# pyannote/pyannote-video

Hardware: AMD Instinct MI355X
Metric: frames/sec end-to-end detect->embed->cluster, 1080p@25fps (higher is better)
Workload: dtype f32 (detector scores, embedder) / f64 (tracker, clustering) / u8 frames; an f16 screening pass with a proven error bound decides which windows the detector's exact f32 chain is evaluated for -- results identical to dense f32 scoring (`dense_scoring`)

## Files before the change

### pyannote-video_amd/csrc/ert.hip

```cpp
#include "pvf_internal.h"

struct ErtJob { const uint8_t* img; int h, w; int rect[4]; };

__global__ void __launch_bounds__(256) ert_k(const ErtJob* __restrict__ jobs, int n_cascades, int n_trees, int n_parts, int n_pix, int depth,
                                             const float* __restrict__ initial, const int32_t* __restrict__ anchor,
                                             const float* __restrict__ deltas, const int32_t* __restrict__ idx1,
                                             const int32_t* __restrict__ idx2, const float* __restrict__ thresh,
                                             const float* __restrict__ leaves, int32_t* __restrict__ pts)
{
    extern __shared__ __attribute__((aligned(16))) float smem[];
    const int P2 = 2 * n_parts;
    float* cur = smem;
    float* pix = cur + ((P2 + 3) & ~3);
    int* leaf = reinterpret_cast<int*>(pix + ((n_pix + 3) & ~3));
    __shared__ float M[4];
    const ErtJob job = jobs[blockIdx.x];
    const int tid = threadIdx.x;
    const int n_split = (1 << depth) - 1, n_leaf = 1 << depth;
    const double sx = (double)job.rect[2] - (double)job.rect[0], sy = (double)job.rect[3] - (double)job.rect[1];
    const double ox = job.rect[0], oy = job.rect[1];
    for (int k = tid; k < P2; k += blockDim.x) cur[k] = initial[k];
    for (int it = 0; it < n_cascades; ++it) {
        __syncthreads();
        if (tid == 0) {
            double mfx = 0, mfy = 0, mtx = 0, mty = 0;
            for (int i = 0; i < n_parts; ++i) { mfx += initial[2 * i]; mfy += initial[2 * i + 1]; mtx += cur[2 * i]; mty += cur[2 * i + 1]; }
            mfx /= n_parts; mfy /= n_parts; mtx /= n_parts; mty /= n_parts;
            double a = 0, b = 0, s = 0;
            for (int i = 0; i < n_parts; ++i) {
                const double fx = initial[2 * i] - mfx, fy = initial[2 * i + 1] - mfy;
                const double tx = cur[2 * i] - mtx, ty = cur[2 * i + 1] - mty;
                a += fx * tx + fy * ty;
                b += fx * ty - fy * tx;
                s += fx * fx + fy * fy;
            }
            const double ca = a / s, cb = b / s;
            M[0] = (float)ca; M[1] = (float)(-cb); M[2] = (float)cb; M[3] = (float)ca;
        }
        __syncthreads();
        const int32_t* an = anchor + (size_t)it * n_pix;
        const float* dl = deltas + (size_t)it * n_pix * 2;
        for (int i = tid; i < n_pix; i += blockDim.x) {
            const float dx = dl[2 * i], dy = dl[2 * i + 1];
            const int ai = an[i];
            const float u = (M[0] * dx + M[1] * dy) + cur[2 * ai];
            const float v = (M[2] * dx + M[3] * dy) + cur[2 * ai + 1];
            const double X = (double)u * sx + ox, Y = (double)v * sy + oy;
            const long px = (long)floor(X + 0.5), py = (long)floor(Y + 0.5);
            float val = 0.0f;
            if (px >= 0 && py >= 0 && px < job.w && py < job.h) {
                const uint8_t* p = job.img + ((size_t)py * job.w + px) * 3;
                val = (float)(((unsigned)p[0] + p[1] + p[2]) / 3);
            }
            pix[i] = val;
        }
        __syncthreads();
        for (int t = tid; t < n_trees; t += blockDim.x) {
            const size_t sb = ((size_t)it * n_trees + t) * n_split;
            int i = 0;
            while (i < n_split) {
                if (pix[idx1[sb + i]] - pix[idx2[sb + i]] > thresh[sb + i]) i = 2 * i + 1;
                else i = 2 * i + 2;
            }
            leaf[t] = i - n_split;
        }
        __syncthreads();
        for (int k = tid; k < P2; k += blockDim.x) {
            float acc = cur[k];
            const float* lb = leaves + (size_t)it * n_trees * n_leaf * P2 + k;
            int t = 0;
            for (; t + 20 <= n_trees; t += 20) {
                float v[20];
#pragma unroll
                for (int j = 0; j < 20; ++j) v[j] = lb[((size_t)(t + j) * n_leaf + leaf[t + j]) * P2];
#pragma unroll
                for (int j = 0; j < 20; ++j) acc = acc + v[j];
            }
            for (; t < n_trees; ++t) acc = acc + lb[((size_t)t * n_leaf + leaf[t]) * P2];
            cur[k] = acc;
        }
    }
    __syncthreads();
    for (int i = tid; i < n_parts; i += blockDim.x) {
        const double X = (double)cur[2 * i] * sx + ox, Y = (double)cur[2 * i + 1] * sy + oy;
        pts[((size_t)blockIdx.x * n_parts + i) * 2] = (int32_t)floor(X + 0.5);
        pts[((size_t)blockIdx.x * n_parts + i) * 2 + 1] = (int32_t)floor(Y + 0.5);
    }
}

void ert_run(Ctx* c, const std::vector<Frame>& frames, const pvf_rect_i32* boxes, int n, int32_t* pts)
{
    const ShapeModel& s = c->shape;
    PVF_REQUIRE(s.loaded, "shape predictor not loaded");
    if (n == 0) return;
    std::vector<ErtJob> jobs(n);
    for (int i = 0; i < n; ++i) {
        jobs[i].img = frames[i].d; jobs[i].h = frames[i].h; jobs[i].w = frames[i].w;
        jobs[i].rect[0] = boxes[i].left; jobs[i].rect[1] = boxes[i].top; jobs[i].rect[2] = boxes[i].right; jobs[i].rect[3] = boxes[i].bottom;
    }
    ScratchLayout lay;
    const auto sJobs = lay.take<ErtJob>(n, 64); const auto sPts = lay.take<int32_t>((size_t)n * s.n_parts * 2, 64);
    lay.pad(64);
    c->s_misc.ensure(lay.bytes());
    ErtJob* d_jobs = sJobs.in(c->s_misc); int32_t* d_pts = sPts.in(c->s_misc);
    HIP_CHECK(hipMemcpyAsync(d_jobs, jobs.data(), sJobs.bytes(), hipMemcpyHostToDevice, c->stream));
    const size_t lds = (size_t)(((2 * s.n_parts + 3) & ~3) + ((s.n_pix + 3) & ~3)) * 4 + (size_t)s.n_trees * 4;
    {
        ProfScope ps(c, "ert");
        hipLaunchKernelGGL(ert_k, dim3(n), dim3(256), lds, c->stream, d_jobs, s.n_cascades, s.n_trees,
                           s.n_parts, s.n_pix, s.depth, s.d_initial, s.d_anchor, s.d_deltas, s.d_idx1, s.d_idx2, s.d_thresh, s.d_leaves,
                           d_pts);
    }
    HIP_CHECK(hipGetLastError());
    HIP_CHECK(hipMemcpyAsync(pts, d_pts, sPts.bytes(), hipMemcpyDeviceToHost, c->stream));
    HIP_CHECK(hipStreamSynchronize(c->stream));
}
```

### pyannote-video_amd/csrc/resnet.hip

```cpp
#include "pvf_internal.h"
#include <cmath>
#include <cstdlib>
#include <cstring>
#include <vector>

typedef float f32x4 __attribute__((ext_vector_type(4)));
typedef uint32_t u32x4 __attribute__((ext_vector_type(4)));
typedef float f32x16 __attribute__((ext_vector_type(16)));
typedef _Float16 f16x8 __attribute__((ext_vector_type(8)));
typedef _Float16 f16x4 __attribute__((ext_vector_type(4)));
typedef uint32_t u32x2 __attribute__((ext_vector_type(2)));

void face_chip_details(const EmbedModel& m, const int32_t* pts, ChipDetails* out)
{
    const double size = m.chip_size, padding = m.chip_padding;
    double fx[51], fy[51], tx[51], ty[51];
    int n = 0;
    for (int i = 17; i < 68; ++i) {
        if ((55 <= i && i <= 59) || (65 <= i && i <= 67)) continue;
        if (17 <= i && i <= 26) continue;
        fx[n] = ((padding + (double)m.mean_shape[2 * (i - 17)]) / (2 * padding + 1)) * size;
        fy[n] = ((padding + (double)m.mean_shape[2 * (i - 17) + 1]) / (2 * padding + 1)) * size;
        tx[n] = pts[2 * i]; ty[n] = pts[2 * i + 1];
        ++n;
    }
    double mfx = 0, mfy = 0, mtx = 0, mty = 0;
    for (int i = 0; i < n; ++i) { mfx += fx[i]; mfy += fy[i]; mtx += tx[i]; mty += ty[i]; }
    mfx /= n; mfy /= n; mtx /= n; mty /= n;
    double a = 0, b = 0, s = 0;
    for (int i = 0; i < n; ++i) {
        const double ax = fx[i] - mfx, ay = fy[i] - mfy, bx = tx[i] - mtx, by = ty[i] - mty;
        a += ax * bx + ay * by;
        b += ax * by - ay * bx;
        s += ax * ax + ay * ay;
    }
    const double ca = a / s, cb = b / s;
    const double scale = std::sqrt(ca * ca + cb * cb);
    const double hx = size / 2.0, hy = size / 2.0;
    const double cx = (ca * (hx - mfx) - cb * (hy - mfy)) + mtx;
    const double cy = (cb * (hx - mfx) + ca * (hy - mfy)) + mty;
    const double wv = size * scale;
    out->l = cx - wv / 2; out->t = cy - wv / 2; out->r = cx + wv / 2; out->b = cy + wv / 2;
    out->cs = ca / scale; out->sn = cb / scale;
    out->rows = m.chip_size; out->cols = m.chip_size;
}

struct ConvArgs {
    const float* in; int B, H, W, Cin;
    const float* w; int K;
    const float* frag;
    const float* bias; const float* gamma; const float* beta;
    float* out; int OH, OW, Cout;
    int AH, AW;
    int ksz, stride, pad;
    int skip_mode;
    const float* skip; int XH, XW, XC, SH, SW;
    const uint32_t* wsplit; float out_scale; int* flags;
};


__device__ __forceinline__ int small_div(int x, int d, float rd)
{
    int q = (int)((float)x * rd);
    const int r = x - q * d;
    q += (r >= d) ? 1 : 0;
    q -= (r < 0) ? 1 : 0;
    return q;
}

template <int WM, int WN>
__device__ __forceinline__ void conv_epilogue(const ConvArgs& a, float* smem, const f32x16& acc0, const f32x16& acc1, long M, long m0, int n0,
                                              int rel0, int b_first, int hw, float r_hw, float r_ow, int wave, int lane)
{
    constexpr int PITCH = 36;
    const int wm = wave / WN, wn = wave % WN;
    const int li = lane & 31, kh = lane >> 5;
    const int col = n0 + wn * 32 + li;
    const float bias = a.bias[col], g = a.gamma[col], bt = a.beta[col];
    if (a.AH == a.OH && a.AW == a.OW && a.skip_mode != 2) {
        float* T = smem + wave * 64 * PITCH;
#pragma unroll
        for (int t = 0; t < 2; ++t)
#pragma unroll
            for (int reg = 0; reg < 16; ++reg)
                T[(t * 32 + (reg & 3) + 8 * (reg >> 2) + 4 * kh) * PITCH + li] = (t == 0 ? acc0[reg] : acc1[reg]);
        __builtin_amdgcn_wave_barrier();
        const int c4 = lane & 7, cb = n0 + wn * 32 + 4 * c4;
        const float4 bias4 = *reinterpret_cast<const float4*>(a.bias + cb), g4 = *reinterpret_cast<const float4*>(a.gamma + cb),
                     bt4 = *reinterpret_cast<const float4*>(a.beta + cb);
#pragma unroll
        for (int it = 0; it < 8; ++it) {
            const int row = it * 8 + (lane >> 3);
            const long m = m0 + wm * 64 + row;
            if (m >= M) continue;
            const float4 x = *reinterpret_cast<const float4*>(&T[row * PITCH + 4 * c4]);
            float4 v = make_float4((x.x + bias4.x) * g4.x + bt4.x, (x.y + bias4.y) * g4.y + bt4.y, (x.z + bias4.z) * g4.z + bt4.z,
                                   (x.w + bias4.w) * g4.w + bt4.w);
            if (a.skip_mode == 1) {
                const float4 sk = *reinterpret_cast<const float4*>(a.skip + (size_t)m * a.Cout + cb);
                v.x += sk.x; v.y += sk.y; v.z += sk.z; v.w += sk.w;
            }
            { v.x = v.x < 0.0f ? 0.0f : v.x; v.y = v.y < 0.0f ? 0.0f : v.y; v.z = v.z < 0.0f ? 0.0f : v.z; v.w = v.w < 0.0f ? 0.0f : v.w; }
            *reinterpret_cast<float4*>(a.out + (size_t)m * a.Cout + cb) = v;
        }
        return;
    }
#pragma unroll
    for (int t = 0; t < 2; ++t)
#pragma unroll
        for (int reg = 0; reg < 16; ++reg) {
            const int row = (reg & 3) + 8 * (reg >> 2) + 4 * kh;
            const long m = m0 + wm * 64 + t * 32 + row;
            if (m >= M) continue;
            const int rel = rel0 + wm * 64 + t * 32 + row;
            const int bb = small_div(rel, hw, r_hw);
            const int rem = rel - bb * hw;
            const int oy = small_div(rem, a.OW, r_ow);
            const int ox = rem - oy * a.OW;
            const int b = b_first + bb;
            float v = 0.0f;
            if (oy < a.AH && ox < a.AW) v = ((t == 0 ? acc0[reg] : acc1[reg]) + bias) * g + bt;
            if (a.skip_mode == 1) v += a.skip[(size_t)m * a.Cout + col];
            else if (a.skip_mode == 2) {
                if (col < a.XC && oy < a.SH && ox < a.SW) {
                    const float* q = a.skip + (((size_t)b * a.XH + 2 * oy) * a.XW + 2 * ox) * a.XC + col;
                    v += (((q[0] + q[a.XC]) + q[(size_t)a.XW * a.XC]) + q[(size_t)a.XW * a.XC + a.XC]) * 0.25f;
                }
            }
            if (v < 0.0f) v = 0.0f;
            a.out[(size_t)m * a.Cout + col] = v;
        }
}

struct ConvExact {
    static constexpr bool FLAGS = false;
    static constexpr int LANE_K = 16;
    static __device__ __forceinline__ const u32x4* weights(const ConvArgs& a) { return reinterpret_cast<const u32x4*>(a.w); }
    static __device__ __forceinline__ bool park_a(uint32_t* row, int j4, const u32x4& v)
    {
        *reinterpret_cast<uint2*>(row + 2 * j4) = make_uint2(v.x, v.z);
        *reinterpret_cast<uint2*>(row + 2 * j4 + 16) = make_uint2(v.y, v.w);
        return true;
    }
    static __device__ __forceinline__ void park_b(uint32_t* row, int j4, const u32x4& v) { park_a(row, j4, v); }
    static __device__ __forceinline__ void chunk(const uint32_t* pa0, const uint32_t* pa1, const uint32_t* pb, f32x16& acc0, f32x16& acc1)
    {
        f32x4 fa0[4], fa1[4], fb[4];
#pragma unroll
        for (int q = 0; q < 4; ++q) {
            fa0[q] = *reinterpret_cast<const f32x4*>(pa0 + 4 * q);
            fa1[q] = *reinterpret_cast<const f32x4*>(pa1 + 4 * q);
            fb[q] = *reinterpret_cast<const f32x4*>(pb + 4 * q);
        }
#pragma unroll
        for (int s = 0; s < 16; ++s) {
            acc0 = __builtin_amdgcn_mfma_f32_32x32x2f32(fa0[s >> 2][s & 3], fb[s >> 2][s & 3], acc0, 0, 0, 0);
            acc1 = __builtin_amdgcn_mfma_f32_32x32x2f32(fa1[s >> 2][s & 3], fb[s >> 2][s & 3], acc1, 0, 0, 0);
        }
    }
    static __device__ __forceinline__ void scale(const ConvArgs&, f32x16&, f32x16&) {}
};

#define EMB_A_SCALE_EXP 8
#define EMB_F16_LIMIT 65504.0f
struct ConvSplit {
    static constexpr bool FLAGS = true;
    static constexpr int LANE_K = 4;
    static __device__ __forceinline__ const u32x4* weights(const ConvArgs& a) { return reinterpret_cast<const u32x4*>(a.wsplit); }
    static __device__ __forceinline__ bool park_a(uint32_t* row, int j4, const u32x4& v)
    {
        const f32x4 xv = __builtin_bit_cast(f32x4, v) * (float)(1 << EMB_A_SCALE_EXP);
        const bool ok = __builtin_reduce_and(__builtin_elementwise_abs(xv) < EMB_F16_LIMIT);
        const f16x4 hi = __builtin_convertvector(xv, f16x4), lo = __builtin_convertvector(xv - __builtin_convertvector(hi, f32x4), f16x4);
        *reinterpret_cast<u32x2*>(row + 2 * j4) = __builtin_bit_cast(u32x2, hi);
        *reinterpret_cast<u32x2*>(row + 2 * j4 + 16) = __builtin_bit_cast(u32x2, lo);
        return ok;
    }
    static __device__ __forceinline__ void park_b(uint32_t* row, int j4, const u32x4& v) { *reinterpret_cast<u32x4*>(row + 4 * j4) = v; }
    static __device__ __forceinline__ void chunk(const uint32_t* pa0, const uint32_t* pa1, const uint32_t* pb, f32x16& acc0, f32x16& acc1)
    {
#pragma unroll
        for (int s = 0; s < 2; ++s) {
            const f16x8 ah0 = *reinterpret_cast<const f16x8*>(pa0 + 8 * s), al0 = *reinterpret_cast<const f16x8*>(pa0 + 16 + 8 * s);
            const f16x8 ah1 = *reinterpret_cast<const f16x8*>(pa1 + 8 * s), al1 = *reinterpret_cast<const f16x8*>(pa1 + 16 + 8 * s);
            const f16x8 bh = *reinterpret_cast<const f16x8*>(pb + 8 * s), bl = *reinterpret_cast<const f16x8*>(pb + 16 + 8 * s);
            acc0 = __builtin_amdgcn_mfma_f32_32x32x16_f16(ah0, bh, acc0, 0, 0, 0);
            acc1 = __builtin_amdgcn_mfma_f32_32x32x16_f16(ah1, bh, acc1, 0, 0, 0);
            acc0 = __builtin_amdgcn_mfma_f32_32x32x16_f16(ah0, bl, acc0, 0, 0, 0);
            acc1 = __builtin_amdgcn_mfma_f32_32x32x16_f16(ah1, bl, acc1, 0, 0, 0);
            acc0 = __builtin_amdgcn_mfma_f32_32x32x16_f16(al0, bh, acc0, 0, 0, 0);
            acc1 = __builtin_amdgcn_mfma_f32_32x32x16_f16(al1, bh, acc1, 0, 0, 0);
        }
    }
    static __device__ __forceinline__ void scale(const ConvArgs& a, f32x16& acc0, f32x16& acc1) { acc0 *= a.out_scale; acc1 *= a.out_scale; }
};

template <int WM, int WN, class Ops>
__global__ void __launch_bounds__(256) conv_tile_k(ConvArgs a)
{
    constexpr int BM = 64 * WM, BN = 32 * WN, KC = 32, PITCH = 36;
    static_assert(WM * WN == 4, "four waves per block");
    constexpr int SM_ROWS = (BM + BN > 256) ? BM + BN : 256;
    __shared__ __attribute__((aligned(16))) float smem[SM_ROWS * PITCH];
    uint32_t* As = reinterpret_cast<uint32_t*>(smem);
    uint32_t* Bs = As + BM * PITCH;
    const int tid = threadIdx.x, lane = tid & 63, wave = tid >> 6;
    const int wm = wave / WN, wn = wave % WN;
    const long M = (long)a.B * a.OH * a.OW;
    const long m0 = (long)blockIdx.x * BM;
    const int n0 = blockIdx.y * BN;
    f32x16 acc0, acc1;
#pragma unroll
    for (int i = 0; i < 16; ++i) { acc0[i] = 0.0f; acc1[i] = 0.0f; }

    constexpr int A_F4 = BM * 8 / 256, B_F4 = BN * 8 / 256;
    constexpr int RSRC_FLAGS = 0x00020000, OOB = (int)0x80000000;
    const int hw = a.OH * a.OW;
    const int b_first = (int)(m0 / hw);
    const int rel0 = (int)(m0 - (long)b_first * hw);
    const float r_hw = 1.0f / (float)hw, r_ow = 1.0f / (float)a.OW;
    const size_t face = (size_t)a.H * a.W * a.Cin;
    const size_t in_bytes = (size_t)(a.B - b_first) * face * sizeof(float);
    const __amdgpu_buffer_rsrc_t rs_in = __builtin_amdgcn_make_buffer_rsrc((void*)(a.in + (size_t)b_first * face), 0,
                                                                           in_bytes > 0x7ffffff0u ? 0x7ffffff0 : (int)in_bytes, RSRC_FLAGS);
    int pa_off[A_F4], pa_y[A_F4], pa_x[A_F4];
#pragma unroll
    for (int q = 0; q < A_F4; ++q) {
        const int i = (tid + q * 256) >> 3;
        const long m = m0 + i;
        pa_off[q] = 0; pa_y[q] = -(1 << 20); pa_x[q] = 0;
        if (m < M) {
            const int rel = rel0 + i;
            const int bb = small_div(rel, hw, r_hw);
            const int rem = rel - bb * hw;
            const int oy = small_div(rem, a.OW, r_ow);
            const int ox = rem - oy * a.OW;
            if (oy < a.AH && ox < a.AW) {
                pa_y[q] = oy * a.stride - a.pad; pa_x[q] = ox * a.stride - a.pad;
                pa_off[q] = ((bb * a.H + pa_y[q]) * a.W + pa_x[q]) * a.Cin;
            }
        }
    }
    const int Kpad = (a.K + KC - 1) / KC * KC;
    const int j4 = tid & 7;
    const u32x4* wrow[B_F4];
#pragma unroll
    for (int q = 0; q < B_F4; ++q) wrow[q] = Ops::weights(a) + (size_t)(n0 + ((tid + q * 256) >> 3)) * (Kpad / 4) + j4;
    u32x4 va[A_F4], vb[B_F4];
    int f_r = 0, f_s = 0, f_c = 0, f_k = 0;
    int voff[A_F4], woff = 0;
    auto offsets = [&]() {
        const int kq = f_k + 4 * j4;
        const int r = f_r, sft = f_s;
        const int delta = (r * a.W + sft) * a.Cin + f_c + 4 * j4;
        const int k_ok = (kq < a.K) ? -1 : 0;
#pragma unroll
        for (int q = 0; q < A_F4; ++q) {
            const int iy = pa_y[q] + r, ix = pa_x[q] + sft;
            const int ok = k_ok & -(int)((unsigned)iy < (unsigned)a.H) & -(int)((unsigned)ix < (unsigned)a.W);
            voff[q] = (((pa_off[q] + delta) * 4) & ok) | (OOB & ~ok);
        }
        woff = f_k >> 2;
        if (f_k + KC < Kpad) {
            f_k += KC;
            f_c += KC;
            if (f_c >= a.Cin) { f_c = 0; if (++f_s == a.ksz) { f_s = 0; ++f_r; } }
        }
    };
    auto issue = [&]() {
#pragma unroll
        for (int q = 0; q < A_F4; ++q) va[q] = __builtin_amdgcn_raw_buffer_load_b128(rs_in, voff[q], 0, 0);
#pragma unroll
        for (int q = 0; q < B_F4; ++q) vb[q] = wrow[q][woff];
    };
    auto park = [&]() {
        int bad = 0;
#pragma unroll
        for (int q = 0; q < A_F4; ++q) bad |= Ops::park_a(&As[((tid + q * 256) >> 3) * PITCH], j4, va[q]) ? 0 : (1 << q);
#pragma unroll
        for (int q = 0; q < B_F4; ++q) Ops::park_b(&Bs[((tid + q * 256) >> 3) * PITCH], j4, vb[q]);
        if constexpr (Ops::FLAGS)
            if (bad)
                for (int q = 0; q < A_F4; ++q)
                    if ((bad >> q) & 1) a.flags[b_first + small_div(rel0 + ((tid + q * 256) >> 3), hw, r_hw)] = 1;
    };
    const int li = lane & 31, kh = lane >> 5;
    const uint32_t* pa0 = &As[(wm * 64 + li) * PITCH + Ops::LANE_K * kh];
    const uint32_t* pa1 = pa0 + 32 * PITCH;
    const uint32_t* pb = &Bs[(wn * 32 + li) * PITCH + Ops::LANE_K * kh];
    offsets();
    issue();
    offsets();
    for (int k0 = 0; k0 < Kpad; k0 += KC) {
        park();
        __syncthreads();
        issue();
        __builtin_amdgcn_sched_barrier(0);
        offsets();
        Ops::chunk(pa0, pa1, pb, acc0, acc1);
        __syncthreads();
    }
    Ops::scale(a, acc0, acc1);
    conv_epilogue<WM, WN>(a, smem, acc0, acc1, M, m0, n0, rel0, b_first, hw, r_hw, r_ow, wave, lane);
}


__global__ void __launch_bounds__(256) conv_wsplit_k(const float* __restrict__ w, int total, int w_exp, _Float16* __restrict__ out)
{
    const int i = blockIdx.x * 256 + threadIdx.x;
    if (i >= total) return;
    const float v = ldexpf(w[i], w_exp);
    const _Float16 hi = (_Float16)v;
    const _Float16 lo = (_Float16)(v - (float)hi);
    const int row32 = i >> 5, kk = i & 31;
    out[(size_t)row32 * 64 + kk] = hi;
    out[(size_t)row32 * 64 + 32 + kk] = lo;
}

__global__ void __launch_bounds__(64) embed_probe_k(const uint4* __restrict__ a, const uint4* __restrict__ b, int steps, float* __restrict__ d)
{
    const int lane = threadIdx.x;
    f32x16 acc;
#pragma unroll
    for (int i = 0; i < 16; ++i) acc[i] = 0.0f;
    for (int s = 0; s < steps; ++s)
        acc = __builtin_amdgcn_mfma_f32_32x32x16_f16(__builtin_bit_cast(f16x8, a[s * 64 + lane]), __builtin_bit_cast(f16x8, b[s * 64 + lane]), acc, 0, 0, 0);
    for (int i = 0; i < 16; ++i) d[lane * 16 + i] = acc[i];
}

#define STEM_ROWS 4
#define STEM_IN_DW 1464
#define STEM_NP 77
__global__ void __launch_bounds__(64) stem_frag_k(const float* __restrict__ w, float* __restrict__ frag)
{
    const int p = blockIdx.x, l = threadIdx.x;
    const int r = p / 11, t = 2 * (p - r * 11) + (l >> 5);
    frag[p * 64 + l] = (t < 21) ? w[(size_t)(l & 31) * 224 + (r * 7 + t / 3) * 4 + t % 3] : 0.0f;
}

__global__ void __launch_bounds__(192) stem_conv_k(const uint8_t* __restrict__ chips, int B, const float* __restrict__ frag, const float* __restrict__ bias,
                                                   const float* __restrict__ gamma, const float* __restrict__ beta, float* __restrict__ out)
{
    constexpr int S = 150, OW = 72;
    __shared__ uint32_t s_in[STEM_IN_DW];
    __shared__ __attribute__((aligned(16))) float s_b[STEM_NP * 64];
    const int tid = threadIdx.x, lane = tid & 63, wave = tid >> 6;
    const int face = blockIdx.y, oy0 = blockIdx.x * STEM_ROWS;
    {
        const size_t total = (size_t)B * S * S * 3;
        const __amdgpu_buffer_rsrc_t rs = __builtin_amdgcn_make_buffer_rsrc((void*)(chips + (size_t)face * S * S * 3), 0,
                                                                             (int)std::min<size_t>(total - (size_t)face * S * S * 3, 0x7ffffff0u), 0x00020000);
        const int first = 2 * oy0 * S * 3;
        for (int i = tid; i < STEM_IN_DW; i += 192) s_in[i] = __builtin_amdgcn_raw_buffer_load_b32(rs, 4 * i, first, 0);
        const float4* f4 = reinterpret_cast<const float4*>(frag);
        float4* b4 = reinterpret_cast<float4*>(s_b);
        for (int i = tid; i < STEM_NP * 16; i += 192) b4[i] = f4[i];
    }
    __syncthreads();
    const int li = lane & 31, kh = lane >> 5;
    const uint8_t* px = reinterpret_cast<const uint8_t*>(s_in);
    const uint8_t* base[3];
#pragma unroll
    for (int t = 0; t < 3; ++t) {
        const int m = (wave * 3 + t) * 32 + li;
        const int oy = m / OW, ox = m - oy * OW;
        base[t] = px + ((2 * oy) * S + 2 * ox) * 3 + kh;
    }
    const float M0 = 122.782f, M1 = 117.001f, M2 = 104.298f;
    const float mean3[3] = {kh ? M1 : M0, kh ? M0 : M2, kh ? M2 : M1};
    f32x16 acc[3];
#pragma unroll
    for (int t = 0; t < 3; ++t)
#pragma unroll
        for (int i = 0; i < 16; ++i) acc[t][i] = 0.0f;
#pragma unroll
    for (int s = 0; s < STEM_NP; ++s) {
        const int r = s / 11, pp = s - r * 11;
        const int off = r * S * 3 + 2 * pp;
        const float b = s_b[s * 64 + lane];
#pragma unroll
        for (int t = 0; t < 3; ++t) {
            const float a = ((float)base[t][off] - mean3[pp % 3]) / 256.0f;
            acc[t] = __builtin_amdgcn_mfma_f32_32x32x2f32(a, b, acc[t], 0, 0, 0);
        }
    }
    const float bs = bias[li], g = gamma[li], bt = beta[li];
// ... 103 lines not shown
            for (int i = 0; i < 16; ++i) acc[t][i] = 0.0f;
#pragma unroll
        for (int s = 0; s < NP; ++s) {
            const int tap = s >> 4, r = tap / 3, q = tap - r * 3;
            const int off = (r * TW + q) * PITCH + 2 * (s & 15);
            const float b = bl[s * 64];
#pragma unroll
            for (int t = 0; t < 2; ++t) acc[t] = __builtin_amdgcn_mfma_f32_32x32x2f32(base[t][off], b, acc[t], 0, 0, 0);
        }
        const int face = item / 5, oy0 = (item - face * 5) * C32_ROWS;
        const __amdgpu_buffer_rsrc_t ro = __builtin_amdgcn_make_buffer_rsrc((void*)(out + ((size_t)face * HW + oy0) * HW * 32), 0, BAND_BYTES, 0x00020000);
        float x[2][16];
        if (skip) {
#pragma unroll
            for (int t = 0; t < 2; ++t)
#pragma unroll
                for (int reg = 0; reg < 16; ++reg) {
                    const float y = ((acc[t][reg] + bs) * g + bt) + sk[t][reg];
                    x[t][reg] = y < 0.0f ? 0.0f : y;
                }
        } else {
#pragma unroll
            for (int t = 0; t < 2; ++t)
#pragma unroll
                for (int reg = 0; reg < 16; ++reg) {
                    const float y = (acc[t][reg] + bs) * g + bt;
                    x[t][reg] = y < 0.0f ? 0.0f : y;
                }
        }
#pragma unroll
        for (int t = 0; t < 2; ++t)
#pragma unroll
            for (int reg = 0; reg < 16; ++reg)
                __builtin_amdgcn_raw_buffer_store_b32(__builtin_bit_cast(uint32_t, x[t][reg]), ro, e_off[t][reg], 0, 0);
        __syncthreads();
        item = next;
    }
}

__global__ void __launch_bounds__(256) maxpool3s2_k(const float* __restrict__ in, int B, int H, int W, int C, float* __restrict__ out, int OH, int OW)
{
    const size_t i = (size_t)blockIdx.x * blockDim.x + threadIdx.x;
    const size_t total = (size_t)B * OH * OW * C;
    if (i >= total) return;
    const int c = (int)(i % C);
    size_t t = i / C;
    const int ox = (int)(t % OW); t /= OW;
    const int oy = (int)(t % OH);
    const int b = (int)(t / OH);
    float mx = -INFINITY;
    for (int r = 0; r < 3; ++r)
        for (int s = 0; s < 3; ++s) {
            const float v = in[(((size_t)b * H + oy * 2 + r) * W + ox * 2 + s) * C + c];
            mx = fmaxf(mx, v);
        }
    out[i] = mx;
}

__global__ void __launch_bounds__(256) head_k(const float* __restrict__ x, int HW, const float* __restrict__ fc, float* __restrict__ out)
{
    __shared__ float feat[256];
    const int b = blockIdx.x, t = threadIdx.x;
    float s = 0.0f;
    for (int i = 0; i < HW; ++i) s += x[((size_t)b * HW + i) * 256 + t];
    feat[t] = s / (float)HW;
    __syncthreads();
    if (t < 128) {
        float acc = 0.0f;
        for (int o = 0; o < 256; ++o) acc += feat[o] * fc[(size_t)o * 128 + t];
        out[(size_t)b * 128 + t] = acc;
    }
}

static bool conv_is_c32(const ConvArgs& a)
{
    return a.Cin == 32 && a.Cout == 32 && a.H == 35 && a.W == 35 && a.OH == 35 && a.OW == 35 && a.AH == 35 && a.AW == 35 && a.ksz == 3 &&
           a.stride == 1 && a.pad == 1 && a.skip_mode != 2;
}

static void launch_conv(Ctx* c, const ConvArgs& a)
{
    const long M = (long)a.B * a.OH * a.OW;
    PVF_REQUIRE(a.Cin % 32 == 0, "conv: input channels must be a multiple of 32 (the 3-channel first layer has a kernel of its own: stem_conv_k)");
    PVF_REQUIRE(a.OH * a.OW < (1 << 21) && a.Cout % 32 == 0, "conv: output map too large for the kernel's index arithmetic / Cout not a multiple of 32");
    auto tile = [&](auto exact, auto split, dim3 grid) { hipLaunchKernelGGL((a.wsplit ? split : exact), grid, dim3(256), 0, c->stream, a); };
    if (a.frag && conv_is_c32(a)) {
        static std::atomic<uint64_t> attr_set{0};
        const size_t lds = (size_t)(C32_TILE_FLOATS + 144 * 64) * sizeof(float);
        const uint64_t bit = 1ull << (c->device & 63);
        if (!(attr_set.load() & bit)) {
            HIP_CHECK(hipFuncSetAttribute(reinterpret_cast<const void*>(conv3x3_c32_k), hipFuncAttributeMaxDynamicSharedMemorySize, (int)lds));
            attr_set.fetch_or(bit);
        }
        const int items = a.B * (35 / C32_ROWS);
        hipLaunchKernelGGL(conv3x3_c32_k, dim3((unsigned)std::min(items, 2 * c->n_cu)), dim3(256), lds, c->stream, a.in, a.frag, a.bias, a.gamma, a.beta,
                           a.skip_mode == 1 ? a.skip : nullptr, a.out, items);
    } else if (a.Cout == 32) {
        tile(conv_tile_k<4, 1, ConvExact>, conv_tile_k<4, 1, ConvSplit>, dim3((unsigned)((M + 255) / 256), 1));
    } else {
        PVF_REQUIRE(a.Cout % 64 == 0, "conv: Cout must be 32 or a multiple of 64");
        tile(conv_tile_k<2, 2, ConvExact>, conv_tile_k<2, 2, ConvSplit>, dim3((unsigned)((M + 127) / 128), a.Cout / 64));
    }
}

void conv_layer_upload(ConvLayer& L, const float* w, const float* bias, const float* gamma, const float* beta)
{
    const int cin = L.cin, cout = L.cout, k = L.k;
    const int cp = (cin == 3) ? 4 : cin;
    const int K = k * k * cp, Kpad = (K + 31) / 32 * 32;
    std::vector<float> wt((size_t)cout * Kpad, 0.0f);
    for (int o = 0; o < cout; ++o)
        for (int ci = 0; ci < cin; ++ci)
            for (int r = 0; r < k; ++r)
                for (int s = 0; s < k; ++s) {
                    const int kk = (r * k + s) * cp + ci;
                    wt[(size_t)o * Kpad + kk] = w[(((size_t)o * cin + ci) * k + r) * k + s];
                }
    auto up = [](const float* src, size_t count) {
        float* d = nullptr;
        HIP_CHECK(hipMalloc((void**)&d, count * sizeof(float)));
        HIP_CHECK(hipMemcpy(d, src, count * sizeof(float), hipMemcpyHostToDevice));
        return d;
    };
    L.d_w = up(wt.data(), wt.size());
    float wmax = 0.0f;
    for (float v : wt) wmax = std::max(wmax, std::fabs(v));
    int ex = 0;
    if (wmax > 0.0f && std::isfinite(wmax)) { std::frexp(wmax, &ex); L.w_exp = 15 - ex; }
    L.d_bias = up(bias, cout);
    L.d_gamma = up(gamma, cout);
    L.d_beta = up(beta, cout);
}

void conv_layer_free(ConvLayer& L)
{
    for (void* p : {(void*)L.d_w, (void*)L.d_bias, (void*)L.d_gamma, (void*)L.d_beta, (void*)L.d_frag, (void*)L.d_wsplit})
        if (p) (void)hipFree(p);
    L.d_w = L.d_bias = L.d_gamma = L.d_beta = L.d_frag = nullptr;
    L.d_wsplit = nullptr;
}

static void conv_bind_weights(Ctx* c, ConvLayer& L, bool split, bool generic, int* flags, ConvArgs& a)
{
    a.w = L.d_w; a.K = L.k * L.k * L.cin; a.bias = L.d_bias; a.gamma = L.d_gamma; a.beta = L.d_beta;
    a.frag = nullptr; a.wsplit = nullptr; a.out_scale = 0.0f; a.flags = nullptr;
    if (!generic && L.cin == 32 && L.cout == 32 && L.k == 3) {
        if (!conv_is_c32(a)) return;
        if (!L.d_frag) {
            HIP_CHECK(hipMalloc(&L.d_frag, 144 * 64 * sizeof(float)));
            hipLaunchKernelGGL(conv_frag_k, dim3(144), dim3(64), 0, c->stream, L.d_w, 288, L.d_frag);
        }
        a.frag = L.d_frag;
        return;
    }
    if (!split) return;
    if (!L.d_wsplit) {
        const int Kpad = (L.k * L.k * L.cin + 31) / 32 * 32;
        const int total = L.cout * Kpad;
        HIP_CHECK(hipMalloc(&L.d_wsplit, (size_t)total * 2 * sizeof(_Float16)));
        hipLaunchKernelGGL(conv_wsplit_k, dim3((unsigned)((total + 255) / 256)), dim3(256), 0, c->stream, L.d_w, total, L.w_exp,
                           reinterpret_cast<_Float16*>(L.d_wsplit));
    }
    a.wsplit = L.d_wsplit;
    a.out_scale = std::ldexp(1.0f, -(EMB_A_SCALE_EXP + L.w_exp));
    a.flags = flags;
}

static uint16_t f16_bits(float v)
{
    const _Float16 h = (_Float16)v;
    uint16_t u;
    memcpy(&u, &h, 2);
    return u;
}

static void embed_probe(Ctx* c)
{
    const int steps = 144;
    const int K = steps * 16;
    const size_t nh = (size_t)steps * 64 * 8;
    std::vector<uint16_t> ha(nh), hb(nh);
    std::vector<double> A((size_t)32 * K), B((size_t)K * 32);
    uint8_t* dev = nullptr;
// ... 255 lines not shown
```

Measured before the change: 4816.

## Double-buffer ERT leaf rows into LDS with async global_load_lds, pair tree walks

Gathers the selected leaf-delta rows for each chunk of 32 trees into a double-buffered LDS tile using the global_load_lds builtin, so the next chunk's loads overlap the current chunk's accumulation. Before this, each thread gathered its column through strided, dependent global reads. The change also processes two pixels and two trees per thread iteration to expose more independent memory loads. In exchange it uses more LDS, adds a size guard, and relies on explicit vmcnt waits and lane-relative LDS addressing that must match the hardware semantics.

```diff
diff --git a/pyannote-video_amd/csrc/ert.hip b/pyannote-video_amd/csrc/ert.hip
--- a/pyannote-video_amd/csrc/ert.hip
+++ b/pyannote-video_amd/csrc/ert.hip
@@ -1,6 +1,34 @@
 #include "pvf_internal.h"
 
 struct ErtJob { const uint8_t* img; int h, w; int rect[4]; };
+
+#define ERT_CHUNK 32
+
+static inline size_t ert_lds_bytes(int n_parts, int n_pix, int n_trees)
+{
+    return (size_t)(((2 * n_parts + 3) & ~3) + ((n_pix + 3) & ~3) + ((n_trees + 3) & ~3) + 2 * ERT_CHUNK * 2 * n_parts) * 4;
+}
+
+template <int PB>
+__device__ __forceinline__ void ert_stage_rows(const float* __restrict__ lcas, const int* leaf, float* tile, int t0, int rows, int P2,
+                                               int n_leaf)
+{
+    const int ppr = P2 * 4 / PB;
+    const int n_pieces = rows * ppr;
+    const int lane = threadIdx.x & 63;
+    const int dq = 256 / ppr, dr = 256 % ppr;
+    int row = (int)threadIdx.x / ppr, j = (int)threadIdx.x % ppr;
+    for (int p = threadIdx.x; p < n_pieces; p += 256) {
+        const int t = t0 + row;
+        const float* src = lcas + ((size_t)t * n_leaf + leaf[t]) * P2 + j * (PB / 4);
+        const __attribute__((address_space(1))) void* g = (const __attribute__((address_space(1))) void*)src;
+        __attribute__((address_space(3))) void* l = (__attribute__((address_space(3))) void*)(tile + (size_t)(p - lane) * (PB / 4));
+        if constexpr (PB == 16) __builtin_amdgcn_global_load_lds(g, l, 16, 0, 0);
+        else __builtin_amdgcn_global_load_lds(g, l, 4, 0, 0);
+        row += dq; j += dr;
+        if (j >= ppr) { j -= ppr; ++row; }
+    }
+}
 
 __global__ void __launch_bounds__(256) ert_k(const ErtJob* __restrict__ jobs, int n_cascades, int n_trees, int n_parts, int n_pix, int depth,
                                              const float* __restrict__ initial, const int32_t* __restrict__ anchor,
@@ -13,12 +41,15 @@
     float* cur = smem;
     float* pix = cur + ((P2 + 3) & ~3);
     int* leaf = reinterpret_cast<int*>(pix + ((n_pix + 3) & ~3));
+    float* tile = reinterpret_cast<float*>(leaf + ((n_trees + 3) & ~3));
     __shared__ float M[4];
     const ErtJob job = jobs[blockIdx.x];
     const int tid = threadIdx.x;
     const int n_split = (1 << depth) - 1, n_leaf = 1 << depth;
     const double sx = (double)job.rect[2] - (double)job.rect[0], sy = (double)job.rect[3] - (double)job.rect[1];
     const double ox = job.rect[0], oy = job.rect[1];
+    const bool wide = (P2 & 3) == 0;
+    const int n_chunks = (n_trees + ERT_CHUNK - 1) / ERT_CHUNK;
     for (int k = tid; k < P2; k += blockDim.x) cur[k] = initial[k];
     for (int it = 0; it < n_cascades; ++it) {
         __syncthreads();
@@ -40,44 +71,68 @@
         __syncthreads();
         const int32_t* an = anchor + (size_t)it * n_pix;
         const float* dl = deltas + (size_t)it * n_pix * 2;
-        for (int i = tid; i < n_pix; i += blockDim.x) {
-            const float dx = dl[2 * i], dy = dl[2 * i + 1];
-            const int ai = an[i];
-            const float u = (M[0] * dx + M[1] * dy) + cur[2 * ai];
-            const float v = (M[2] * dx + M[3] * dy) + cur[2 * ai + 1];
-            const double X = (double)u * sx + ox, Y = (double)v * sy + oy;
-            const long px = (long)floor(X + 0.5), py = (long)floor(Y + 0.5);
-            float val = 0.0f;
-            if (px >= 0 && py >= 0 && px < job.w && py < job.h) {
-                const uint8_t* p = job.img + ((size_t)py * job.w + px) * 3;
-                val = (float)(((unsigned)p[0] + p[1] + p[2]) / 3);
+        for (int i0 = tid; i0 < n_pix; i0 += 2 * blockDim.x) {
+            float val[2];
+            const uint8_t* p[2];
+            bool in[2];
+#pragma unroll
+            for (int u = 0; u < 2; ++u) {
+                const int i = min(i0 + u * (int)blockDim.x, n_pix - 1);
+                const float dx = dl[2 * i], dy = dl[2 * i + 1];
+                const int ai = an[i];
+                const float uu = (M[0] * dx + M[1] * dy) + cur[2 * ai];
+                const float v = (M[2] * dx + M[3] * dy) + cur[2 * ai + 1];
+                const double X = (double)uu * sx + ox, Y = (double)v * sy + oy;
+                const long px = (long)floor(X + 0.5), py = (long)floor(Y + 0.5);
+                in[u] = px >= 0 && py >= 0 && px < job.w && py < job.h;
+                p[u] = job.img + (in[u] ? ((size_t)py * job.w + px) * 3 : (size_t)0);
             }
-            pix[i] = val;
+#pragma unroll
+            for (int u = 0; u < 2; ++u) val[u] = (float)(((unsigned)p[u][0] + p[u][1] + p[u][2]) / 3);
+            pix[i0] = in[0] ? val[0] : 0.0f;
+            if (i0 + (int)blockDim.x < n_pix) pix[i0 + blockDim.x] = in[1] ? val[1] : 0.0f;
         }
         __syncthreads();
-        for (int t = tid; t < n_trees; t += blockDim.x) {
-            const size_t sb = ((size_t)it * n_trees + t) * n_split;
-            int i = 0;
-            while (i < n_split) {
-                if (pix[idx1[sb + i]] - pix[idx2[sb + i]] > thresh[sb + i]) i = 2 * i + 1;
+        for (int t0 = tid; t0 < n_trees; t0 += 2 * blockDim.x) {
+            const int t1 = t0 + blockDim.x;
+            const size_t sb0 = ((size_t)it * n_trees + t0) * n_split, sb1 = ((size_t)it * n_trees + min(t1, n_trees - 1)) * n_split;
+            int i = 0, i2 = 0;
+            for (int d = 0; d < depth; ++d) {
+                const int a1 = idx1[sb0 + i], a2 = idx2[sb0 + i], b1 = idx1[sb1 + i2], b2 = idx2[sb1 + i2];
+                const float ta = thresh[sb0 + i], tb = thresh[sb1 + i2];
+                if (pix[a1] - pix[a2] > ta) i = 2 * i + 1;
                 else i = 2 * i + 2;
+                if (pix[b1] - pix[b2] > tb) i2 = 2 * i2 + 1;
+                else i2 = 2 * i2 + 2;
             }
-            leaf[t] = i - n_split;
+            leaf[t0] = i - n_split;
+            if (t1 < n_trees) leaf[t1] = i2 - n_split;
         }
         __syncthreads();
-        for (int k = tid; k < P2; k += blockDim.x) {
-            float acc = cur[k];
-            const float* lb = leaves + (size_t)it * n_trees * n_leaf * P2 + k;
-            int t = 0;
-            for (; t + 20 <= n_trees; t += 20) {
-                float v[20];
+        const float* lcas = leaves + (size_t)it * n_trees * n_leaf * P2;
+        if (wide) ert_stage_rows<16>(lcas, leaf, tile, 0, min(ERT_CHUNK, n_trees), P2, n_leaf);
+        else ert_stage_rows<4>(lcas, leaf, tile, 0, min(ERT_CHUNK, n_trees), P2, n_leaf);
+        for (int c = 0; c < n_chunks; ++c) {
+            asm volatile("s_waitcnt vmcnt(0)" ::: "memory");
+            __syncthreads();
+            if (c + 1 < n_chunks) {
+                const int t0 = (c + 1) * ERT_CHUNK, rows = min(ERT_CHUNK, n_trees - t0);
+                float* dst = tile + (size_t)((c + 1) & 1) * ERT_CHUNK * P2;
+                if (wide) ert_stage_rows<16>(lcas, leaf, dst, t0, rows, P2, n_leaf);
+                else ert_stage_rows<4>(lcas, leaf, dst, t0, rows, P2, n_leaf);
+            }
+            const float* src = tile + (size_t)(c & 1) * ERT_CHUNK * P2;
+            const int rows = min(ERT_CHUNK, n_trees - c * ERT_CHUNK);
+            for (int k = tid; k < P2; k += blockDim.x) {
+                float acc = cur[k];
+                if (rows == ERT_CHUNK) {
 #pragma unroll
-                for (int j = 0; j < 20; ++j) v[j] = lb[((size_t)(t + j) * n_leaf + leaf[t + j]) * P2];
-#pragma unroll
-                for (int j = 0; j < 20; ++j) acc = acc + v[j];
+                    for (int r = 0; r < ERT_CHUNK; ++r) acc = acc + src[r * P2 + k];
+                } else {
+                    for (int r = 0; r < rows; ++r) acc = acc + src[r * P2 + k];
+                }
+                cur[k] = acc;
             }
-            for (; t < n_trees; ++t) acc = acc + lb[((size_t)t * n_leaf + leaf[t]) * P2];
-            cur[k] = acc;
         }
     }
     __syncthreads();
@@ -104,7 +159,8 @@
     c->s_misc.ensure(lay.bytes());
     ErtJob* d_jobs = sJobs.in(c->s_misc); int32_t* d_pts = sPts.in(c->s_misc);
     HIP_CHECK(hipMemcpyAsync(d_jobs, jobs.data(), sJobs.bytes(), hipMemcpyHostToDevice, c->stream));
-    const size_t lds = (size_t)(((2 * s.n_parts + 3) & ~3) + ((s.n_pix + 3) & ~3)) * 4 + (size_t)s.n_trees * 4;
+    const size_t lds = ert_lds_bytes(s.n_parts, s.n_pix, s.n_trees);
+    PVF_REQUIRE(lds <= 64 * 1024, "shape predictor too large for the landmark kernel's LDS");
     {
         ProfScope ps(c, "ert");
         hipLaunchKernelGGL(ert_k, dim3(n), dim3(256), lds, c->stream, d_jobs, s.n_cascades, s.n_trees,
```

Result: no change. 4795 (-0.4%).

## Widen split-f16 conv tile to two column tiles per wave, buffer-load weights

Applied to the files above, without the earlier changes.

For split-f16 convolutions with Cout a multiple of 128, each wave now computes two 32-column output tiles, so every A fragment is reused across twice as many MFMAs and half as many blocks are launched. Weight loads move to buffer-resource loads. The per-element f16 range check becomes a running integer max of magnitudes that is checked once after the K loop. The general epilogue now stages accumulators through shared memory, and pixel coordinates are packed into 16-bit pairs to save registers. The wider tile doubles the accumulator registers per wave, which raises register pressure, and launch_bounds now also requests a minimum of 3 blocks per multiprocessor.

```diff
diff --git a/pyannote-video_amd/csrc/resnet.hip b/pyannote-video_amd/csrc/resnet.hip
--- a/pyannote-video_amd/csrc/resnet.hip
+++ b/pyannote-video_amd/csrc/resnet.hip
@@ -77,14 +77,14 @@
     const int li = lane & 31, kh = lane >> 5;
     const int col = n0 + wn * 32 + li;
     const float bias = a.bias[col], g = a.gamma[col], bt = a.beta[col];
+    float* T = smem + wave * 64 * PITCH;
+#pragma unroll
+    for (int t = 0; t < 2; ++t)
+#pragma unroll
+        for (int reg = 0; reg < 16; ++reg)
+            T[(t * 32 + (reg & 3) + 8 * (reg >> 2) + 4 * kh) * PITCH + li] = (t == 0 ? acc0[reg] : acc1[reg]);
+    __builtin_amdgcn_wave_barrier();
     if (a.AH == a.OH && a.AW == a.OW && a.skip_mode != 2) {
-        float* T = smem + wave * 64 * PITCH;
-#pragma unroll
-        for (int t = 0; t < 2; ++t)
-#pragma unroll
-            for (int reg = 0; reg < 16; ++reg)
-                T[(t * 32 + (reg & 3) + 8 * (reg >> 2) + 4 * kh) * PITCH + li] = (t == 0 ? acc0[reg] : acc1[reg]);
-        __builtin_amdgcn_wave_barrier();
         const int c4 = lane & 7, cb = n0 + wn * 32 + 4 * c4;
         const float4 bias4 = *reinterpret_cast<const float4*>(a.bias + cb), g4 = *reinterpret_cast<const float4*>(a.gamma + cb),
                      bt4 = *reinterpret_cast<const float4*>(a.beta + cb);
@@ -105,46 +105,45 @@
         }
         return;
     }
-#pragma unroll
-    for (int t = 0; t < 2; ++t)
-#pragma unroll
-        for (int reg = 0; reg < 16; ++reg) {
-            const int row = (reg & 3) + 8 * (reg >> 2) + 4 * kh;
-            const long m = m0 + wm * 64 + t * 32 + row;
-            if (m >= M) continue;
-            const int rel = rel0 + wm * 64 + t * 32 + row;
-            const int bb = small_div(rel, hw, r_hw);
-            const int rem = rel - bb * hw;
-            const int oy = small_div(rem, a.OW, r_ow);
-            const int ox = rem - oy * a.OW;
-            const int b = b_first + bb;
-            float v = 0.0f;
-            if (oy < a.AH && ox < a.AW) v = ((t == 0 ? acc0[reg] : acc1[reg]) + bias) * g + bt;
-            if (a.skip_mode == 1) v += a.skip[(size_t)m * a.Cout + col];
-            else if (a.skip_mode == 2) {
-                if (col < a.XC && oy < a.SH && ox < a.SW) {
-                    const float* q = a.skip + (((size_t)b * a.XH + 2 * oy) * a.XW + 2 * ox) * a.XC + col;
-                    v += (((q[0] + q[a.XC]) + q[(size_t)a.XW * a.XC]) + q[(size_t)a.XW * a.XC + a.XC]) * 0.25f;
-                }
+#pragma unroll 2
+    for (int e = 0; e < 32; ++e) {
+        const int row = 2 * e + kh;
+        const long m = m0 + wm * 64 + row;
+        if (m >= M) continue;
+        const int rel = rel0 + wm * 64 + row;
+        const int bb = small_div(rel, hw, r_hw);
+        const int rem = rel - bb * hw;
+        const int oy = small_div(rem, a.OW, r_ow);
+        const int ox = rem - oy * a.OW;
+        const int b = b_first + bb;
+        float v = 0.0f;
+        if (oy < a.AH && ox < a.AW) v = (T[row * PITCH + li] + bias) * g + bt;
+        if (a.skip_mode == 1) v += a.skip[(size_t)m * a.Cout + col];
+        else if (a.skip_mode == 2) {
+            if (col < a.XC && oy < a.SH && ox < a.SW) {
+                const float* q = a.skip + (((size_t)b * a.XH + 2 * oy) * a.XW + 2 * ox) * a.XC + col;
+                v += (((q[0] + q[a.XC]) + q[(size_t)a.XW * a.XC]) + q[(size_t)a.XW * a.XC + a.XC]) * 0.25f;
             }
-            if (v < 0.0f) v = 0.0f;
-            a.out[(size_t)m * a.Cout + col] = v;
-        }
+        }
+        if (v < 0.0f) v = 0.0f;
+        a.out[(size_t)m * a.Cout + col] = v;
+    }
 }
 
 struct ConvExact {
     static constexpr bool FLAGS = false;
     static constexpr int LANE_K = 16;
     static __device__ __forceinline__ const u32x4* weights(const ConvArgs& a) { return reinterpret_cast<const u32x4*>(a.w); }
-    static __device__ __forceinline__ bool park_a(uint32_t* row, int j4, const u32x4& v)
+    static __device__ __forceinline__ void park_a(uint32_t* row, int j4, const u32x4& v, uint32_t&)
     {
         *reinterpret_cast<uint2*>(row + 2 * j4) = make_uint2(v.x, v.z);
         *reinterpret_cast<uint2*>(row + 2 * j4 + 16) = make_uint2(v.y, v.w);
-        return true;
-    }
-    static __device__ __forceinline__ void park_b(uint32_t* row, int j4, const u32x4& v) { park_a(row, j4, v); }
-    static __device__ __forceinline__ void chunk(const uint32_t* pa0, const uint32_t* pa1, const uint32_t* pb, f32x16& acc0, f32x16& acc1)
+    }
+    static __device__ __forceinline__ void park_b(uint32_t* row, int j4, const u32x4& v) { uint32_t none = 0; park_a(row, j4, v, none); }
+    template <int WC>
+    static __device__ __forceinline__ void chunk(const uint32_t* pa0, const uint32_t* pa1, const uint32_t* pb, f32x16 (&acc)[2 * WC])
     {
+        static_assert(WC == 1, "the exact form runs on the one-column wave tile");
         f32x4 fa0[4], fa1[4], fb[4];
 #pragma unroll
         for (int q = 0; q < 4; ++q) {
@@ -154,52 +153,67 @@
         }
 #pragma unroll
         for (int s = 0; s < 16; ++s) {
-            acc0 = __builtin_amdgcn_mfma_f32_32x32x2f32(fa0[s >> 2][s & 3], fb[s >> 2][s & 3], acc0, 0, 0, 0);
-            acc1 = __builtin_amdgcn_mfma_f32_32x32x2f32(fa1[s >> 2][s & 3], fb[s >> 2][s & 3], acc1, 0, 0, 0);
-        }
-    }
-    static __device__ __forceinline__ void scale(const ConvArgs&, f32x16&, f32x16&) {}
+            acc[0] = __builtin_amdgcn_mfma_f32_32x32x2f32(fa0[s >> 2][s & 3], fb[s >> 2][s & 3], acc[0], 0, 0, 0);
+            acc[1] = __builtin_amdgcn_mfma_f32_32x32x2f32(fa1[s >> 2][s & 3], fb[s >> 2][s & 3], acc[1], 0, 0, 0);
+        }
+    }
+    template <int N>
+    static __device__ __forceinline__ void scale(const ConvArgs&, f32x16 (&)[N]) {}
 };
 
 #define EMB_A_SCALE_EXP 8
-#define EMB_F16_LIMIT 65504.0f
 struct ConvSplit {
     static constexpr bool FLAGS = true;
     static constexpr int LANE_K = 4;
     static __device__ __forceinline__ const u32x4* weights(const ConvArgs& a) { return reinterpret_cast<const u32x4*>(a.wsplit); }
-    static __device__ __forceinline__ bool park_a(uint32_t* row, int j4, const u32x4& v)
+    static constexpr uint32_t RANGE_LIMIT_BITS = 0x437fe000u;
+    static_assert(EMB_A_SCALE_EXP == 8, "RANGE_LIMIT_BITS is 65504 / 2^EMB_A_SCALE_EXP");
+    static __device__ __forceinline__ void park_a(uint32_t* row, int j4, const u32x4& v, uint32_t& amax)
     {
         const f32x4 xv = __builtin_bit_cast(f32x4, v) * (float)(1 << EMB_A_SCALE_EXP);
-        const bool ok = __builtin_reduce_and(__builtin_elementwise_abs(xv) < EMB_F16_LIMIT);
+        const u32x4 mag = v & 0x7fffffffu;
+        amax = max(max(max(max(amax, mag.x), mag.y), mag.z), mag.w);
         const f16x4 hi = __builtin_convertvector(xv, f16x4), lo = __builtin_convertvector(xv - __builtin_convertvector(hi, f32x4), f16x4);
         *reinterpret_cast<u32x2*>(row + 2 * j4) = __builtin_bit_cast(u32x2, hi);
         *reinterpret_cast<u32x2*>(row + 2 * j4 + 16) = __builtin_bit_cast(u32x2, lo);
-        return ok;
     }
     static __device__ __forceinline__ void park_b(uint32_t* row, int j4, const u32x4& v) { *reinterpret_cast<u32x4*>(row + 4 * j4) = v; }
-    static __device__ __forceinline__ void chunk(const uint32_t* pa0, const uint32_t* pa1, const uint32_t* pb, f32x16& acc0, f32x16& acc1)
+    template <int WC>
+    static __device__ __forceinline__ void chunk(const uint32_t* pa0, const uint32_t* pa1, const uint32_t* pb, f32x16 (&acc)[2 * WC])
     {
+        constexpr int PITCH = 36;
 #pragma unroll
         for (int s = 0; s < 2; ++s) {
-            const f16x8 ah0 = *reinterpret_cast<const f16x8*>(pa0 + 8 * s), al0 = *reinterpret_cast<const f16x8*>(pa0 + 16 + 8 * s);
-            const f16x8 ah1 = *reinterpret_cast<const f16x8*>(pa1 + 8 * s), al1 = *reinterpret_cast<const f16x8*>(pa1 + 16 + 8 * s);
-            const f16x8 bh = *reinterpret_cast<const f16x8*>(pb + 8 * s), bl = *reinterpret_cast<const f16x8*>(pb + 16 + 8 * s);
-            acc0 = __builtin_amdgcn_mfma_f32_32x32x16_f16(ah0, bh, acc0, 0, 0, 0);
-            acc1 = __builtin_amdgcn_mfma_f32_32x32x16_f16(ah1, bh, acc1, 0, 0, 0);
-            acc0 = __builtin_amdgcn_mfma_f32_32x32x16_f16(ah0, bl, acc0, 0, 0, 0);
-            acc1 = __builtin_amdgcn_mfma_f32_32x32x16_f16(ah1, bl, acc1, 0, 0, 0);
-            acc0 = __builtin_amdgcn_mfma_f32_32x32x16_f16(al0, bh, acc0, 0, 0, 0);
-            acc1 = __builtin_amdgcn_mfma_f32_32x32x16_f16(al1, bh, acc1, 0, 0, 0);
-        }
-    }
-    static __device__ __forceinline__ void scale(const ConvArgs& a, f32x16& acc0, f32x16& acc1) { acc0 *= a.out_scale; acc1 *= a.out_scale; }
+            f16x8 ah[2], al[2], bh[WC], bl[WC];
+            ah[0] = *reinterpret_cast<const f16x8*>(pa0 + 8 * s); al[0] = *reinterpret_cast<const f16x8*>(pa0 + 16 + 8 * s);
+            ah[1] = *reinterpret_cast<const f16x8*>(pa1 + 8 * s); al[1] = *reinterpret_cast<const f16x8*>(pa1 + 16 + 8 * s);
+#pragma unroll
+            for (int c = 0; c < WC; ++c) {
+                bh[c] = *reinterpret_cast<const f16x8*>(pb + c * 32 * PITCH + 8 * s);
+                bl[c] = *reinterpret_cast<const f16x8*>(pb + c * 32 * PITCH + 16 + 8 * s);
+            }
+#pragma unroll
+            for (int term = 0; term < 3; ++term)
+#pragma unroll
+                for (int c = 0; c < WC; ++c)
+#pragma unroll
+                    for (int t = 0; t < 2; ++t)
+                        acc[t * WC + c] = __builtin_amdgcn_mfma_f32_32x32x16_f16(term == 2 ? al[t] : ah[t], term == 1 ? bl[c] : bh[c], acc[t * WC + c], 0, 0, 0);
+        }
+    }
+    template <int N>
+    static __device__ __forceinline__ void scale(const ConvArgs& a, f32x16 (&acc)[N])
+    {
+#pragma unroll
+        for (int i = 0; i < N; ++i) acc[i] *= a.out_scale;
+    }
 };
 
-template <int WM, int WN, class Ops>
-__global__ void __launch_bounds__(256) conv_tile_k(ConvArgs a)
-{
-    constexpr int BM = 64 * WM, BN = 32 * WN, KC = 32, PITCH = 36;
-    static_assert(WM * WN == 4, "four waves per block");
+template <int WM, int WN, class Ops, int WC = 1>
+__global__ void __launch_bounds__(256, 3) conv_tile_k(ConvArgs a)
+{
+    constexpr int BM = 64 * WM, BN = 32 * WN * WC, KC = 32, PITCH = 36;
+    static_assert(WM * WN == 4 && (WC == 1 || WC == 2), "four waves per block, one or two column tiles per wave");
     constexpr int SM_ROWS = (BM + BN > 256) ? BM + BN : 256;
     __shared__ __attribute__((aligned(16))) float smem[SM_ROWS * PITCH];
     uint32_t* As = reinterpret_cast<uint32_t*>(smem);
@@ -209,9 +223,11 @@
     const long M = (long)a.B * a.OH * a.OW;
     const long m0 = (long)blockIdx.x * BM;
     const int n0 = blockIdx.y * BN;
-    f32x16 acc0, acc1;
-#pragma unroll
-    for (int i = 0; i < 16; ++i) { acc0[i] = 0.0f; acc1[i] = 0.0f; }
+    f32x16 acc[2 * WC];
+#pragma unroll
+    for (int t = 0; t < 2 * WC; ++t)
+#pragma unroll
+        for (int i = 0; i < 16; ++i) acc[t][i] = 0.0f;
 
     constexpr int A_F4 = BM * 8 / 256, B_F4 = BN * 8 / 256;
     constexpr int RSRC_FLAGS = 0x00020000, OOB = (int)0x80000000;
@@ -223,12 +239,12 @@
     const size_t in_bytes = (size_t)(a.B - b_first) * face * sizeof(float);
     const __amdgpu_buffer_rsrc_t rs_in = __builtin_amdgcn_make_buffer_rsrc((void*)(a.in + (size_t)b_first * face), 0,
                                                                            in_bytes > 0x7ffffff0u ? 0x7ffffff0 : (int)in_bytes, RSRC_FLAGS);
-    int pa_off[A_F4], pa_y[A_F4], pa_x[A_F4];
+    int pa_off[A_F4], pa_yx[A_F4];
 #pragma unroll
     for (int q = 0; q < A_F4; ++q) {
         const int i = (tid + q * 256) >> 3;
         const long m = m0 + i;
-        pa_off[q] = 0; pa_y[q] = -(1 << 20); pa_x[q] = 0;
+        pa_off[q] = 0; pa_yx[q] = (int)(0xffffc000u << 16);
         if (m < M) {
             const int rel = rel0 + i;
             const int bb = small_div(rel, hw, r_hw);
@@ -236,17 +252,20 @@
             const int oy = small_div(rem, a.OW, r_ow);
             const int ox = rem - oy * a.OW;
             if (oy < a.AH && ox < a.AW) {
-                pa_y[q] = oy * a.stride - a.pad; pa_x[q] = ox * a.stride - a.pad;
-                pa_off[q] = ((bb * a.H + pa_y[q]) * a.W + pa_x[q]) * a.Cin;
+                const int y = oy * a.stride - a.pad, x = ox * a.stride - a.pad;
+                pa_yx[q] = (int)(((unsigned)y << 16) | ((unsigned)x & 0xffffu));
+                pa_off[q] = ((bb * a.H + y) * a.W + x) * a.Cin;
             }
         }
     }
     const int Kpad = (a.K + KC - 1) / KC * KC;
     const int j4 = tid & 7;
-    const u32x4* wrow[B_F4];
-#pragma unroll
-    for (int q = 0; q < B_F4; ++q) wrow[q] = Ops::weights(a) + (size_t)(n0 + ((tid + q * 256) >> 3)) * (Kpad / 4) + j4;
+    const __amdgpu_buffer_rsrc_t rs_w = __builtin_amdgcn_make_buffer_rsrc((void*)(Ops::weights(a) + (size_t)n0 * (Kpad / 4)), 0, BN * Kpad * 4, RSRC_FLAGS);
+    const int wv = ((tid >> 3) * (Kpad / 4) + j4) * 16, wstep = 32 * (Kpad / 4) * 16;
     u32x4 va[A_F4], vb[B_F4];
+    uint32_t amax[A_F4];
+#pragma unroll
+    for (int q = 0; q < A_F4; ++q) amax[q] = 0;
     int f_r = 0, f_s = 0, f_c = 0, f_k = 0;
     int voff[A_F4], woff = 0;
     auto offsets = [&]() {
@@ -256,11 +275,11 @@
         const int k_ok = (kq < a.K) ? -1 : 0;
 #pragma unroll
         for (int q = 0; q < A_F4; ++q) {
-            const int iy = pa_y[q] + r, ix = pa_x[q] + sft;
+            const int iy = (pa_yx[q] >> 16) + r, ix = (int)(short)pa_yx[q] + sft;
             const int ok = k_ok & -(int)((unsigned)iy < (unsigned)a.H) & -(int)((unsigned)ix < (unsigned)a.W);
             voff[q] = (((pa_off[q] + delta) * 4) & ok) | (OOB & ~ok);
         }
-        woff = f_k >> 2;
+        woff = f_k * 4;
         if (f_k + KC < Kpad) {
             f_k += KC;
             f_c += KC;
@@ -271,23 +290,18 @@
 #pragma unroll
         for (int q = 0; q < A_F4; ++q) va[q] = __builtin_amdgcn_raw_buffer_load_b128(rs_in, voff[q], 0, 0);
 #pragma unroll
-        for (int q = 0; q < B_F4; ++q) vb[q] = wrow[q][woff];
+        for (int q = 0; q < B_F4; ++q) vb[q] = __builtin_amdgcn_raw_buffer_load_b128(rs_w, wv, woff + q * wstep, 0);
     };
     auto park = [&]() {
-        int bad = 0;
-#pragma unroll
-        for (int q = 0; q < A_F4; ++q) bad |= Ops::park_a(&As[((tid + q * 256) >> 3) * PITCH], j4, va[q]) ? 0 : (1 << q);
+#pragma unroll
+        for (int q = 0; q < A_F4; ++q) Ops::park_a(&As[((tid + q * 256) >> 3) * PITCH], j4, va[q], amax[q]);
 #pragma unroll
         for (int q = 0; q < B_F4; ++q) Ops::park_b(&Bs[((tid + q * 256) >> 3) * PITCH], j4, vb[q]);
-        if constexpr (Ops::FLAGS)
-            if (bad)
-                for (int q = 0; q < A_F4; ++q)
-                    if ((bad >> q) & 1) a.flags[b_first + small_div(rel0 + ((tid + q * 256) >> 3), hw, r_hw)] = 1;
     };
     const int li = lane & 31, kh = lane >> 5;
     const uint32_t* pa0 = &As[(wm * 64 + li) * PITCH + Ops::LANE_K * kh];
     const uint32_t* pa1 = pa0 + 32 * PITCH;
-    const uint32_t* pb = &Bs[(wn * 32 + li) * PITCH + Ops::LANE_K * kh];
+    const uint32_t* pb = &Bs[(wn * 32 * WC + li) * PITCH + Ops::LANE_K * kh];
     offsets();
     issue();
     offsets();
@@ -297,11 +311,23 @@
         issue();
         __builtin_amdgcn_sched_barrier(0);
         offsets();
-        Ops::chunk(pa0, pa1, pb, acc0, acc1);
+        Ops::template chunk<WC>(pa0, pa1, pb, acc);
         __syncthreads();
     }
-    Ops::scale(a, acc0, acc1);
-    conv_epilogue<WM, WN>(a, smem, acc0, acc1, M, m0, n0, rel0, b_first, hw, r_hw, r_ow, wave, lane);
+    if constexpr (Ops::FLAGS) {
+#pragma unroll
+        for (int q = 0; q < A_F4; ++q)
+            if (amax[q] >= Ops::RANGE_LIMIT_BITS) a.flags[b_first + small_div(rel0 + ((tid + q * 256) >> 3), hw, r_hw)] = 1;
+    }
+    Ops::scale(a, acc);
+#pragma unroll 1
+    for (int c = 0; c < WC; ++c) {
+        conv_epilogue<WM, WN>(a, smem, acc[0], acc[WC], M, m0, n0 + 32 * (WC - 1) * wn + 32 * c, rel0, b_first, hw, r_hw, r_ow, wave, lane);
+        if constexpr (WC > 1) {
+            acc[0] = acc[1]; acc[WC] = acc[WC + 1];
+            __builtin_amdgcn_wave_barrier();
+        }
+    }
 }
 
 
@@ -571,6 +597,8 @@
 {
     const long M = (long)a.B * a.OH * a.OW;
     PVF_REQUIRE(a.Cin % 32 == 0, "conv: input channels must be a multiple of 32 (the 3-channel first layer has a kernel of its own: stem_conv_k)");
+    PVF_REQUIRE(a.H < (1 << 13) && a.W < (1 << 13) && a.stride >= 1 && a.stride <= 4 && a.pad >= 0 && a.pad < 8 && a.ksz >= 1 && a.ksz <= 8,
+                "conv: input map, stride, padding or kernel size beyond the kernel's 16-bit pixel coordinates");
     PVF_REQUIRE(a.OH * a.OW < (1 << 21) && a.Cout % 32 == 0, "conv: output map too large for the kernel's index arithmetic / Cout not a multiple of 32");
     auto tile = [&](auto exact, auto split, dim3 grid) { hipLaunchKernelGGL((a.wsplit ? split : exact), grid, dim3(256), 0, c->stream, a); };
     if (a.frag && conv_is_c32(a)) {
@@ -588,6 +616,10 @@
         tile(conv_tile_k<4, 1, ConvExact>, conv_tile_k<4, 1, ConvSplit>, dim3((unsigned)((M + 255) / 256), 1));
     } else {
         PVF_REQUIRE(a.Cout % 64 == 0, "conv: Cout must be 32 or a multiple of 64");
+        if (a.wsplit && a.Cout % 128 == 0) {
+            hipLaunchKernelGGL((conv_tile_k<2, 2, ConvSplit, 2>), dim3((unsigned)((M + 127) / 128), a.Cout / 128), dim3(256), 0, c->stream, a);
+            return;
+        }
         tile(conv_tile_k<2, 2, ConvExact>, conv_tile_k<2, 2, ConvSplit>, dim3((unsigned)((M + 127) / 128), a.Cout / 64));
     }
 }
```

Result: no change. 4865 before, 4823 after (-0.8%).
